# rfonod/geo-trax

Hardware: AMD Instinct MI355X
Metric: 4K frames/sec through detect+stabilize+track (higher is better)
Workload: dtype f32 (split-f16x3 MFMA)

## Files before the change

### geo-trax_amd/csrc/detector.cpp

```cpp
#include "detector.hpp"
#include "split_format.hpp"

#include <algorithm>
#include <cmath>

namespace gtx {

Detector::Detector(gtx_ctx* ctx, const gtx_det_config& cfg)
    : DetectorBase(ctx, cfg, cfg.half ? DT_F16 : (cfg.fp32_split ? DT_F32S : DT_F32), dtype_size(cfg.half ? DT_F16 : DT_F32),
                   cfg.half ? DT_F16 : DT_F32),
      trunk_(*this, ops_, cfg.half ? DT_F16 : DT_F32) {
  dtype_ = cfg.half ? DT_F16 : DT_F32;
  es_ = dtype_size(dtype_);
  lb_ = letterbox_geometry(cfg.frame_h, cfg.frame_w, cfg.imgsz, cfg.rect != 0, 32);
  GTX_CHECK(lb_.net_h % 32 == 0 && lb_.net_w % 32 == 0, "network input %dx%d is not stride aligned", lb_.net_h, lb_.net_w);
}

Detector::~Detector() {
  if (h_feats_) (void)hipHostFree(h_feats_);
  if (h_count_) (void)hipHostFree(h_count_);
}

std::unique_ptr<NetRuntime> Detector::make_exact() const {
  gtx_det_config c = cfg_;
// ... 16 lines not shown
  const YoloTrunk::Levels trunk = trunk_.build(img_);
  const std::vector<View>& lvl_in = trunk.in;
  const std::vector<float>& strides = trunk.strides;
  det_pfx_ = trunk.det_pfx;
  const int nl = (int)lvl_in.size();
  GTX_CHECK(nl <= kMaxLevels, "internal: %d Detect levels", nl);
  const bool has_o2o = has(det_pfx_ + ".one2one_cv2.0.0.conv.weight");
  end2end_ = cfg_.end2end != 0;
  GTX_CHECK(!end2end_ || has_o2o, "end2end: the checkpoint has no one-to-one head (%s.one2one_cv2 / one2one_cv3): only a YOLOv10 file has", det_pfx_.c_str());
  GTX_CHECK(!end2end_ || !cfg_.obj_feats, "end2end: obj_feats (ReID `model: auto`) is not implemented for the one-to-one head");
  const std::string box_br = end2end_ ? ".one2one_cv2." : ".cv2.", cls_br = end2end_ ? ".one2one_cv3." : ".cv3.";
  GTX_CHECK(has(det_pfx_ + box_br + "0.0.conv.weight") && has(det_pfx_ + cls_br + "0.2.weight"),
            "%s: the checkpoint holds no %s / %s tensors (a fused YOLOv10 export keeps the one-to-one head only: run it with end2end)", det_pfx_.c_str(),
            box_br.substr(1, box_br.size() - 2).c_str(), cls_br.substr(1, cls_br.size() - 2).c_str());

  std::vector<Op> st1, st2;
  const bool dw_cls = trunk.dw_cls;
  std::vector<Op> dw_a, pw_a, dw_b;
  head_ = HeadParams{};
  head_.n_levels = nl;
  head_.nc = cfg_.nc;
  head_.conf = cfg_.conf;
  head_.class_mask[0] = head_.class_mask[1] = cfg_.n_classes == 0 ? ~0ull : 0ull;
  for (int i = 0; i < cfg_.n_classes; ++i)
    if (cfg_.classes[i] >= 0 && cfg_.classes[i] < 128) head_.class_mask[cfg_.classes[i] >> 6] |= 1ull << (cfg_.classes[i] & 63);
  int anchor = 0;
  for (int l = 0; l < nl; ++l) {
    const std::string b2 = det_pfx_ + box_br + std::to_string(l), b3 = det_pfx_ + cls_br + std::to_string(l);
    const HostTensor &w20 = tensor(b2 + ".0.conv.weight"), &w30 = tensor(b3 + (dw_cls ? ".1.1.conv.weight" : ".0.conv.weight"));
    const int cb = (int)w20.shape[0], cc = (int)w30.shape[0], cin = (int)w20.shape[1];
    GTX_CHECK(cin == lvl_in[l].c && (dw_cls || (int)w30.shape[1] == cin), "Detect level %d input channels", l);
    Op o1, o2, o3;
// ... 100 lines not shown
      return a.dtype == b.dtype && a.ks == b.ks && a.stride == b.stride && a.bn == b.bn && a.kc == b.kc &&
             a.variant == b.variant && a.th == b.th && a.tw == b.tw;
    };
    auto add = [&](std::vector<Op>& stage, const char* name, const Op& o) {
      for (Op& g : stage)
        if (same(g.cfg, o.cfg) && g.grp.count < kMaxGroup) { g.grp.p[g.grp.count++] = o.grp.p[0]; return; }
      Op g;
      g.kind = Op::CONV;
      g.name = stage.empty() ? std::string(name) : std::string(name) + "." + std::to_string(stage.size());
      g.cfg = o.cfg;
      g.grp.p[g.grp.count++] = o.grp.p[0];
      stage.push_back(g);
    };
    std::vector<Op> d1, d2;
    for (int l = 0; l < nl; ++l) {
      Op o1 = head_ops_[l][0];
      const Op &o2 = head_ops_[l][1], &o3 = head_ops_[l][2];
      if (sparse_on_) {
        const ConvProblem full = o1.grp.p[0];
        const int cb = head_.lv[l].cb, cc = head_.lv[l].cc;
        const size_t tile_bytes = (size_t)(full.Cin / o1.cfg.kc) * 9 * 64 * 128;
        SparseBoxLevel& S = sparse_.lv[l];
        S.in = full.in; S.H = full.H; S.W = full.W; S.cstride = full.in_cstride; S.coff = full.in_coff; S.cin = full.Cin;
        S.w1 = full.wpack; S.b1 = full.bias; S.sc1 = full.acc_scale;
        S.w2 = o2.grp.p[0].wpack; S.b2 = o2.grp.p[0].bias; S.sc2 = o2.grp.p[0].acc_scale;
        S.anchor_begin = head_.lv[l].anchor_begin;
        S.wb = head_.lv[l].wb; S.bb = head_.lv[l].bb; S.stride = head_.lv[l].stride;
        GTX_CHECK(full.bias && o2.grp.p[0].bias && o2.grp.p[0].Cin == 64 && o2.grp.p[0].Cout == 64, "sparse box branch: unexpected Detect box layers");
        Op box1 = o1;
        box1.grp.p[0].Cout = cb;
        add(d1, (det_pfx_ + ".box1").c_str(), box1);
        add(d2, (det_pfx_ + ".box2").c_str(), o2);
        if (dw_cls) {
          add(st1, (det_pfx_ + ".stage1").c_str(), pw_a[l]);
          add(st2, (det_pfx_ + ".stage2").c_str(), o3);
          continue;
        }
        ConvProblem& p = o1.grp.p[0];
        p.wpack = static_cast<const char*>(full.wpack) + tile_bytes;
        p.bias = full.bias + 64;
        p.Cout = cc;
        p.out_coff = full.out_coff + cb;
        add(st1, (det_pfx_ + ".stage1").c_str(), o1);
        add(st2, (det_pfx_ + ".stage2").c_str(), o3);
      } else {
        if (dw_cls) add(st1, (det_pfx_ + ".stage1").c_str(), pw_a[l]);
        add(st1, (det_pfx_ + ".stage1").c_str(), o1);
        add(st2, (det_pfx_ + ".stage2").c_str(), o2);
        add(st2, (det_pfx_ + ".stage2").c_str(), o3);
      }
    }
    if (sparse_on_) {
      sparse_.n_levels = nl;
      for (std::vector<Op>* stage : {&d1, &d2})
        for (Op& g : *stage) { g.family = conv_kernel_name(g.cfg); dense_box_ops_.push_back(g); }
    }
  }
  feat_levels_ = FeatLevels{};
  if (cfg_.obj_feats) {
    feat_levels_.n_levels = nl;
    feat_levels_.dim = lvl_in[0].c;
    for (int l = 1; l < nl; ++l) feat_levels_.dim = std::min(feat_levels_.dim, lvl_in[l].c);
    for (int l = 0; l < nl; ++l) {
      feat_levels_.feat[l] = lvl_in[l].ptr; feat_levels_.h[l] = lvl_in[l].h; feat_levels_.w[l] = lvl_in[l].w;
      feat_levels_.cstride[l] = lvl_in[l].cstride; feat_levels_.coff[l] = lvl_in[l].coff; feat_levels_.c[l] = lvl_in[l].c;
      feat_levels_.anchor_begin[l] = head_.lv[l].anchor_begin;
      GTX_CHECK(lvl_in[l].c % feat_levels_.dim == 0, "obj_feats: Detect input %d has %d channels, not a multiple of %d", l, lvl_in[l].c, feat_levels_.dim);
    }
  }
  for (std::vector<Op>* stage : {&st1, &st2}) {
    for (const Op& d : stage == &st1 ? dw_a : dw_b) ops_.push_back(d);
    for (Op& g : *stage) {
      g.family = conv_kernel_name(g.cfg);
      ops_.push_back(g);
    }
  }
}

void Detector::set_batch(int nb) {
  if (nb == cur_nb_) return;
  set_batch_ops(ops_, nb, es_, pad_skip_on_);
  cur_nb_ = nb;
}

void Detector::plan_pad_skip() {
  pad_skip_rows_ = pad_skip_total_ = 0;
  struct Rows { int lo, hi; };
  std::map<const void*, Rows> dep;
  std::set<const void*> full;
  struct Writer { int c0, c1; Op* op; int member; };
  std::map<const void*, std::vector<Writer>> writers;
// ... 301 lines not shown
```

### geo-trax_amd/csrc/detector.hpp

```cpp
#pragma once
#include <map>
#include <memory>
#include <set>
#include <string>
#include <vector>

#include "yolo_trunk.hpp"

namespace gtx {

class Detector : public DetectorBase {
 public:
  Detector(gtx_ctx* ctx, const gtx_det_config& cfg);
  ~Detector() override;
  void finalize() override;
  void raw_output(int b, float* out, int* n_anchors, bool logits = false) override;
  void layer_output(int b, const std::string& layer, float* out, int* h, int* w, int* c) override;
  void features(int b, float* out, int cap, int* n, int* dim) const override;
  void pad_skip(int* on, int* skipped, int* total) const override {
    if (on) *on = (!exact_ && pad_skip_on_) ? 1 : 0;
    if (skipped) *skipped = pad_skip_rows_;
    if (total) *total = pad_skip_total_;
  }
  void sparse_box(int* on, int* overflows) const override {
    if (on) *on = (!exact_ && sparse_on_) ? 1 : 0;
    if (overflows) *overflows = sparse_overflows_;
  }

 private:
  size_t op_count() const override { return ops_.size(); }
  const OpInfo& op_info(size_t i) const override { return ops_[i]; }
  void launch_op(size_t i, int nb, hipStream_t s) override { run_op(ops_[i], nb, s); }
  std::unique_ptr<NetRuntime> make_exact() const override;
  void release_graph() override { ops_.clear(); trunk_.clear(); }
  View head_conv(const std::string& name, const View& x, const View* out_slice);
  void build_graph();
  void run_op(const Op& op, int nb, hipStream_t s);
  void run_post(int nb, hipStream_t s) override;
  void after_pass(int nb) override;
  void set_batch(int nb) override;

  int dtype_;
  size_t es_;
  std::vector<Op> ops_;
  YoloTrunk trunk_;
  int force_kc_ = 0;
  int force_bn_ = 0;
// ... 1 lines not shown
  HeadParams head_{};
  NmsBuffers nms_{};
  bool end2end_ = false;
  NmsBuffers sel_{};
  float* v10_scores_ = nullptr;
  static constexpr int kSelCap = 304;
  DevBuf raw_;
  bool plain_out_ = false;
  FeatLevels feat_levels_{};
  static constexpr int kSparseCap = 8192;
  bool sparse_on_ = false;
  SparseBox sparse_{};
  Op head_ops_[kMaxLevels][3];
  std::string det_pfx_ = "model.22";
  std::vector<Op> dense_box_ops_;
  bool dense_head_valid_ = false;
  int* h_count_ = nullptr;
  int sparse_overflows_ = 0;
  void run_dense_box(hipStream_t s);
  bool pad_skip_on_ = false;
  int pad_skip_rows_ = 0, pad_skip_total_ = 0;
  void plan_pad_skip();
  void prime_pad_skip();
  float* d_feats_ = nullptr;
  float* h_feats_ = nullptr;
  std::vector<float> c_feats_;
  std::vector<int> c_feat_n_;
};

}
// ... 1 lines not shown
```

### geo-trax_amd/csrc/gtx_api.cpp

```cpp
#include <chrono>
#include <cmath>
#include <cstring>
#include <memory>
#include <string>

#include "../../include/gtx.h"
#include "api_guard.hpp"
#include "common.hpp"
#include "detector.hpp"
#include "draw.hpp"
#include "rtdetr.hpp"
#include "geometry.hpp"
#include "ecc.hpp"
#include "gmc.hpp"
#include "gmc_feat.hpp"
#include "jpeg.hpp"
#include "jpeg_enc.hpp"
#include "jpeg_entropy.hpp"
#include "register.hpp"
#include "sift.hpp"
#include "sift_stab.hpp"
#include "stabilizer.hpp"
#include "tracker.hpp"

// ... 384 lines not shown
                            float* conf, int* cls, float speed_ms[3]) {
  return guarded([&] {
    need(det, "det"); need(frame_dptr, "frame"); need(n_out, "n_out"); need(xyxy, "xyxy"); need(conf, "conf"); need(cls, "cls");
    det->impl->live()->detect_dev(frame_dptr, 1, h, w, n_out, xyxy, conf, cls, speed_ms);
  });
}
int gtx_detector_detect_batch_dev(gtx_detector* det, const void* frames_dptr, int nb, int h, int w, int* n_out,
                                  float* xyxy, float* conf, int* cls, float speed_ms[3]) {
  return guarded([&] {
    need(det, "det"); need(frames_dptr, "frames"); need(n_out, "n_out"); need(xyxy, "xyxy"); need(conf, "conf"); need(cls, "cls");
    det->impl->live()->detect_dev(frames_dptr, nb, h, w, n_out, xyxy, conf, cls, speed_ms);
  });
}
int gtx_detector_submit_dev(gtx_detector* det, const void* frames_dptr, int nb, int h, int w) {
  return guarded([&] { need(det, "det"); need(frames_dptr, "frames"); det->impl->live()->submit_dev(frames_dptr, nb, h, w); });
}
int gtx_detector_collect(gtx_detector* det, int* n_out, float* xyxy, float* conf, int* cls, float speed_ms[3]) {
  return guarded([&] {
    need(det, "det"); need(n_out, "n_out"); need(xyxy, "xyxy"); need(conf, "conf"); need(cls, "cls");
    det->impl->live()->collect(n_out, xyxy, conf, cls, speed_ms);
  });
}
const void* gtx_detector_gray(gtx_detector* det, int b, int* gray_h, int* gray_w) {
  if (!det) return nullptr;
  return det->impl->live()->gray(b, gray_h, gray_w);
}
int gtx_detector_raw_output(gtx_detector* det, int b, float* out, int* n_anchors) {
  return guarded([&] { need(det, "det"); need(out, "out"); det->impl->live()->raw_output(b, out, n_anchors); });
}
int gtx_detector_raw_logits(gtx_detector* det, int b, float* out, int* n_anchors) {
// ... 580 lines not shown
```

### geo-trax_amd/csrc/net_runtime.cpp

```cpp
#include "net_runtime.hpp"
#include "split_format.hpp"

#include <array>
#include <deque>
#include <functional>
#include <mutex>

namespace gtx {

void KernelTable::add(const std::string& label, int n, float t, double f, double b) {
  auto it = idx.find(label);
  size_t k;
  if (it == idx.end()) {
    k = names.size();
    idx[label] = k;
    names.push_back(label);
    launches.push_back(0); ms.push_back(0.f); flops.push_back(0.0); bytes.push_back(0.0);
  } else {
    k = it->second;
  }
  launches[k] += n;
  ms[k] += t;
  flops[k] += f;
  bytes[k] += b;
}

NetRuntime::~NetRuntime() {
  if (h_sat_) (void)hipHostFree(h_sat_);
}

void NetRuntime::set_tensor(const std::string& name, const float* data, int ndim, const int64_t* shape) {
  GTX_CHECK(!finalized_, "set_tensor after finalize");
  HostTensor t;
  size_t n = 1;
  for (int i = 0; i < ndim; ++i) {
    t.shape.push_back(shape[i]);
    n *= (size_t)shape[i];
  }
  t.data.assign(data, data + n);
  tensors_[name] = std::move(t);
}

// ... 38 lines not shown
}

View NetRuntime::new_view(int h, int w, int c, bool plain) {
  View v;
  v.n = max_batch_;
  v.h = h;
  v.w = w;
  v.cstride = c;
  v.coff = 0;
  v.c = c;
  v.plain = plain;
  v.ptr = alloc((size_t)v.n * h * w * c * view_es_);
  return v;
}

void NetRuntime::run_ops(int nb, hipStream_t s, hipEvent_t* ev) {
  const size_t n = op_count();
  for (size_t i = 0; i < n; ++i) {
    if (ev) GTX_HIP(hipEventRecord(ev[i], s));
    launch_op(i, nb, s);
  }
  if (ev) GTX_HIP(hipEventRecord(ev[n], s));
}

namespace {
struct PackedWeights {
  std::vector<uint8_t> bytes;
  float acc_scale = 1.f;
  std::vector<float> source;
};
std::shared_ptr<const PackedWeights> packed_weights(const float* w, size_t n, int cout, int cin, const ConvConfig& cfg,
                                                    const std::function<PackedWeights()>& make) {
  static std::mutex mu;
  static std::map<std::array<uint64_t, 4>, std::shared_ptr<const PackedWeights>> cache;
  uint64_t h = 1469598103934665603ull;
  const uint64_t* q = reinterpret_cast<const uint64_t*>(w);
  for (size_t i = 0; i < n / 2; ++i) h = (h ^ q[i]) * 1099511628211ull;
// ... 196 lines not shown
  GTX_HIP(hipSetDevice(ctx_->device));
  GTX_HIP(hipEventSynchronize(ev_[3]));
  in_flight_ = false;
  collected_gray_slot_ = gray_slot_;
  if (h_sat_ && *h_sat_) {
    sat_seen_ = true;
    if (can_fall_back()) {
      flight_traced_ = false;
      fall_back_to_exact();
      if (trace_every_ > 0) live()->set_trace(trace_every_);
      return live()->detect_dev(cur_frames_, flight_nb_, cfg_.frame_h, cfg_.frame_w, n_out, xyxy, conf, cls, speed_ms);
    }
  }
  if (flight_traced_) {
    for (size_t i = 0; i < op_count(); ++i) {
      float t = 0.f;
      GTX_HIP(hipEventElapsedTime(&t, trace_ev_[i], trace_ev_[i + 1]));
      trace_ms_[i] += t;
      trace_n_[i] += 1;
      trace_flops_[i] += op_info(i).flops;
      trace_bytes_[i] += op_info(i).bytes;
    }
    flight_traced_ = false;
  }
  after_pass(flight_nb_);
  for (int b = 0; b < flight_nb_; ++b) {
    const int n = h_out_n_[b];
    n_out[b] = n;
    const float* rows = h_out_rows_ + (size_t)b * cfg_.max_det * 6;
    for (int i = 0; i < n; ++i) {
      float* bx = xyxy + ((size_t)b * cfg_.max_det + i) * 4;
      bx[0] = rows[i * 6 + 0]; bx[1] = rows[i * 6 + 1]; bx[2] = rows[i * 6 + 2]; bx[3] = rows[i * 6 + 3];
      conf[(size_t)b * cfg_.max_det + i] = rows[i * 6 + 4];
      cls[(size_t)b * cfg_.max_det + i] = (int)rows[i * 6 + 5];
    }
  }
  if (speed_ms)
    for (int i = 0; i < 3; ++i) GTX_HIP(hipEventElapsedTime(&speed_ms[i], ev_[i], ev_[i + 1]));
}

void DetectorBase::detect_dev(const void* frames, int nb, int h, int w, int* n_out, float* xyxy, float* conf, int* cls, float speed_ms[3]) {
  submit_dev(frames, nb, h, w);
  collect(n_out, xyxy, conf, cls, speed_ms);
}

void DetectorBase::detect_host(const uint8_t* frame, int h, int w, int* n_out, float* xyxy, float* conf, int* cls, float speed_ms[3]) {
  GTX_CHECK(finalized_, "detector not finalized");
  GTX_HIP(hipSetDevice(ctx_->device));
  const size_t bytes = (size_t)h * w * 3;
  if (frame_stage_.bytes < bytes) frame_stage_.alloc(bytes);
  GTX_HIP(hipEventRecord(ev_up_[0], ctx_->stream));
  GTX_HIP(hipMemcpyAsync(frame_stage_.p, frame, bytes, hipMemcpyHostToDevice, ctx_->stream));
  GTX_HIP(hipEventRecord(ev_up_[1], ctx_->stream));
// ... 20 lines not shown
  KernelTable table{names, launches, ms, flops, bytes, {}};
  time_ops(nb, iters, [&](size_t i, float t) {
    const OpInfo& op = op_info(i);
    const std::string n = std::to_string(i);
    table.add(per_op ? std::string(n.size() < 3 ? 3 - n.size() : 0, '0') + n + " " + op.name : op.family, 1, t, op.flops, op.bytes);
  });
}

void DetectorBase::set_trace(int every_n) {
  GTX_CHECK(finalized_ && every_n >= 0, "set_trace: detector not finalized or bad period");
  GTX_CHECK(!in_flight_, "set_trace while a batch is in flight");
  trace_every_ = every_n;
  trace_count_ = 0;
  const size_t n = op_count();
  if (every_n > 0 && trace_ev_.empty()) {
    trace_ev_.resize(n + 1);
    for (auto& e : trace_ev_) GTX_HIP(hipEventCreate(&e));
  }
  trace_ms_.assign(n, 0.0);
  trace_n_.assign(n, 0);
  trace_flops_.assign(n, 0.0);
  trace_bytes_.assign(n, 0.0);
}

void DetectorBase::trace_report(std::vector<std::string>& names, std::vector<int>& launches, std::vector<float>& ms,
                                std::vector<double>& flops, std::vector<double>& bytes) {
  KernelTable table{names, launches, ms, flops, bytes, {}};
  const size_t n = op_count();
  for (size_t i = 0; i < n && i < trace_n_.size(); ++i)
    if (trace_n_[i] > 0) table.add(op_info(i).family, trace_n_[i], (float)trace_ms_[i], trace_flops_[i], trace_bytes_[i]);
  trace_ms_.assign(n, 0.0);
// ... 7 lines not shown
```

### geo-trax_amd/csrc/net_runtime.hpp

```cpp
#pragma once
#include <map>
#include <memory>
#include <string>
#include <vector>

#include "../../include/gtx.h"
#include "common.hpp"
#include "conv_igemm.hpp"
#include "det_kernels.hpp"

struct gtx_ctx {
  int device = 0;
  hipStream_t stream = nullptr;
  hipDeviceProp_t prop{};
  void* orb_op_state = nullptr;
  ~gtx_ctx() {
    if (orb_op_state) (void)hipFree(orb_op_state);
    if (stream) (void)hipStreamDestroy(stream);
  }
};

namespace gtx {

struct HostTensor {
// ... 31 lines not shown
  void add(const std::string& label, int n, float t, double f, double b);
};

class YoloTrunk;

class NetRuntime {
 public:
  NetRuntime(gtx_ctx* ctx, int fmt, size_t view_es, int max_batch) : ctx_(ctx), fmt_(fmt), view_es_(view_es), max_batch_(max_batch) {}
  virtual ~NetRuntime();
  NetRuntime(const NetRuntime&) = delete;
  NetRuntime& operator=(const NetRuntime&) = delete;
  friend class YoloTrunk;
  void set_tensor(const std::string& name, const float* data, int ndim, const int64_t* shape);
  bool saturated(bool clear);
  bool fell_back() const { return exact_ != nullptr; }
  virtual void finalize() = 0;

 protected:
  virtual size_t op_count() const = 0;
  virtual const OpInfo& op_info(size_t i) const = 0;
  virtual void launch_op(size_t i, int nb, hipStream_t s) = 0;
  virtual void set_batch(int nb) = 0;
  void run_ops(int nb, hipStream_t s, hipEvent_t* ev);
  template <class F> void time_ops(int nb, int iters, F fold);

  const HostTensor& tensor(const std::string& name) const;
  bool has(const std::string& name) const { return tensors_.count(name) != 0; }
  const float* bias_of(const std::string& name, int cout) const;
  void* alloc(size_t bytes);
  float* upload(const std::vector<float>& v);
  View new_view(int h, int w, int c, bool plain = false);

  struct ConvArgs {
    int stride = 1, act = 1;
    const View* out_slice = nullptr;
    const View* residual = nullptr;
    bool plain_out = false;
    int force_kc = 0, force_bn = 0;
// ... 39 lines not shown
  gtx_ctx* ctx_;
  int fmt_;
  size_t view_es_;
  int max_batch_;
  bool finalized_ = false;
  int cur_nb_ = 0;
  std::map<std::string, HostTensor> tensors_;
  std::vector<DevBuf> bufs_;
  std::map<std::string, View> layer_views_;
  std::unique_ptr<NetRuntime> exact_;
  int* sat_dev_ = nullptr;
  int* h_sat_ = nullptr;
  bool sat_seen_ = false;

 private:
  View conv_problem(const std::string& name, const float* w_oihw, int cout, int cin, int ks, const float* bias, const View& x,
                    const ConvArgs& a, ConvConfig& cfg, ConvProblem& p);
};

template <class F>
void NetRuntime::time_ops(int nb, int iters, F fold) {
  hipStream_t s = ctx_->stream;
  set_batch(nb);
  const size_t n = op_count();
  std::vector<hipEvent_t> ev(n + 1);
  for (auto& e : ev) GTX_HIP(hipEventCreate(&e));
  for (int it = 0; it < iters; ++it) {
    run_ops(nb, s, ev.data());
    GTX_HIP(hipStreamSynchronize(s));
    for (size_t i = 0; i < n; ++i) {
      float t = 0.f;
      GTX_HIP(hipEventElapsedTime(&t, ev[i], ev[i + 1]));
      fold(i, t);
    }
  }
  for (auto& e : ev) (void)hipEventDestroy(e);
}

class DetectorBase : public NetRuntime {
 public:
  DetectorBase(gtx_ctx* ctx, const gtx_det_config& cfg, int fmt, size_t view_es, int in_dtype);
  ~DetectorBase() override;
  DetectorBase* live() { return live_as<DetectorBase>(); }
  void input_size(int* h, int* w) const { *h = lb_.net_h; *w = lb_.net_w; }
  void detect_dev(const void* frames, int nb, int h, int w, int* n_out, float* xyxy, float* conf, int* cls, float speed_ms[3]);
  void submit_dev(const void* frames, int nb, int h, int w);
  void collect(int* n_out, float* xyxy, float* conf, int* cls, float speed_ms[3]);
  void detect_host(const uint8_t* frame, int h, int w, int* n_out, float* xyxy, float* conf, int* cls, float speed_ms[3]);
  const void* gray(int b, int* gh, int* gw) const;
  virtual void raw_output(int b, float* out, int* n_anchors, bool logits = false) = 0;
  virtual void layer_output(int b, const std::string& layer, float* out, int* h, int* w, int* c) = 0;
  void profile(int nb, int iters, std::vector<std::string>& names, std::vector<int>& launches, std::vector<float>& ms,
               std::vector<double>& flops, std::vector<double>& bytes);
  void set_trace(int every_n);
  void trace_report(std::vector<std::string>& names, std::vector<int>& launches, std::vector<float>& ms, std::vector<double>& flops,
                    std::vector<double>& bytes);
  virtual void features(int b, float* out, int cap, int* n, int* dim) const = 0;
  virtual void pad_skip(int* on, int* skipped, int* total) const = 0;
  virtual void sparse_box(int* on, int* overflows) const = 0;

  static constexpr int kGrayRing = 16;

// ... 37 lines not shown
```

### geo-trax_amd/csrc/yolo_trunk.hpp

```cpp
#pragma once
#include <string>
#include <vector>

#include "net_runtime.hpp"
#include "yolo_tables.hpp"

namespace gtx {

struct Op : OpInfo {
  enum Kind { CONV, STEM, POOL, UPSAMPLE, DWCONV, ATTN, POOLDOWN } kind = CONV;
  ConvGroup grp{};
  ConvConfig cfg{};
  View in, out;
  const float* w27 = nullptr;
  const float* bias = nullptr;
  const void* wpk = nullptr;
  float stem_scale = 1.f;
  const void* front_wpk = nullptr;
  float front_scale = 1.f;
  const float* dw_w = nullptr;
  const float* dw_bias = nullptr;
  int dw_act = 0, heads = 0;
  int dw_k = 3, dw_stride = 1;
  View dw_res;
  View out2;
  int* sat = nullptr;
  int ty_first[kMaxGroup] = {0}, ty_count[kMaxGroup] = {0};
};

void set_batch_ops(std::vector<Op>& ops, int nb, size_t es, bool pad_skip_on);

class YoloTrunk {
 public:
  YoloTrunk(NetRuntime& net, std::vector<Op>& ops, int dtype) : net_(net), ops_(ops), dtype_(dtype) {}

  struct Levels {
    std::vector<View> in;
    std::vector<float> strides;
    std::string det_pfx;
    bool dw_cls = false;
  };
  TrunkGraph choose_graph() const;
// ... 41 lines not shown
```

### geo-trax_amd/geotrax_amd/_lib.py

```python
from __future__ import annotations

import ctypes as C
import os
from pathlib import Path

import numpy as np

_HERE = Path(__file__).resolve().parent
LIB_PATH = Path(os.environ.get("GTX_LIB", _HERE / "libgtx.so"))


class GtxError(RuntimeError):
    def __init__(self, code: int, msg: str):
        super().__init__(f"libgtx error {code}: {msg}")
        self.code = code


class ConvDesc(C.Structure):
    _fields_ = [(n, C.c_int) for n in (
        "dtype", "n", "h", "w", "cin", "cout", "ksize", "stride", "act",
        "in_cstride", "in_coff", "out_cstride", "out_coff", "has_residual")]


class ConvFused(C.Structure):
# ... 183 lines not shown
    "gtx_sift_stab_keypoints": (C.c_int, [_P, C.c_int, C.c_int, C.POINTER(C.c_int), _P, _P, _P]),
    "gtx_sift_stab_pairs": (C.c_int, [_P, C.c_int, C.POINTER(C.c_int), _P]),
    "gtx_sift_stab_counters": (C.c_int, [_P, _P]),
    "gtx_op_match_2nn": (C.c_int, [_P, _P, C.c_int, _P, C.c_int, _P, _P, _P, _P, C.c_int, _P]),
    "gtx_op_preprocess": (C.c_int, [_P, C.c_int, _P, C.c_int, C.c_int, C.c_int, C.c_int, _P, _P, C.c_int, C.c_int]),
    "gtx_detector_create": (C.c_int, [_P, C.POINTER(DetConfig), C.POINTER(_P)]),
    "gtx_detector_destroy": (None, [_P]),
    "gtx_detector_set_tensor": (C.c_int, [_P, C.c_char_p, _P, C.c_int, C.POINTER(C.c_int64)]),
    "gtx_detector_finalize": (C.c_int, [_P]),
    "gtx_detector_input_size": (C.c_int, [_P, C.POINTER(C.c_int), C.POINTER(C.c_int)]),
    "gtx_detector_detect": (C.c_int, [_P, _P, C.c_int, C.c_int, _P, _P, _P, _P, _P]),
    "gtx_detector_detect_dev": (C.c_int, [_P, _P, C.c_int, C.c_int, _P, _P, _P, _P, _P]),
    "gtx_detector_detect_batch_dev": (C.c_int, [_P, _P, C.c_int, C.c_int, C.c_int, _P, _P, _P, _P, _P]),
    "gtx_detector_submit_dev": (C.c_int, [_P, _P, C.c_int, C.c_int, C.c_int]),
    "gtx_detector_collect": (C.c_int, [_P, _P, _P, _P, _P, _P]),
    "gtx_detector_gray": (_P, [_P, C.c_int, C.POINTER(C.c_int), C.POINTER(C.c_int)]),
    "gtx_detector_raw_output": (C.c_int, [_P, C.c_int, _P, C.POINTER(C.c_int)]),
    "gtx_detector_raw_logits": (C.c_int, [_P, C.c_int, _P, C.POINTER(C.c_int)]),
    "gtx_detector_layer_output": (C.c_int, [_P, C.c_int, C.c_char_p, _P, C.POINTER(C.c_int), C.POINTER(C.c_int), C.POINTER(C.c_int)]),
    "gtx_detector_saturated": (C.c_int, [_P, C.c_int, C.POINTER(C.c_int)]),
    "gtx_detector_fell_back": (C.c_int, [_P, C.POINTER(C.c_int)]),
    "gtx_detector_pad_skip": (C.c_int, [_P, C.POINTER(C.c_int), C.POINTER(C.c_int), C.POINTER(C.c_int)]),
    "gtx_detector_sparse_box": (C.c_int, [_P, C.POINTER(C.c_int), C.POINTER(C.c_int)]),
    "gtx_detector_features": (C.c_int, [_P, C.c_int, _P, C.c_int, C.POINTER(C.c_int), C.POINTER(C.c_int)]),
    "gtx_detector_trace": (C.c_int, [_P, C.c_int]),
    "gtx_detector_profile": (C.c_int, [_P, C.c_int, C.c_int, C.c_int, _P, _P, _P, _P, _P, C.POINTER(C.c_int)]),
    "gtx_embedder_create": (C.c_int, [_P, C.c_int, C.c_int, C.c_int, C.POINTER(_P)]),
    "gtx_embedder_destroy": (None, [_P]),
    "gtx_embedder_set_tensor": (C.c_int, [_P, C.c_char_p, _P, C.c_int, C.POINTER(C.c_int64)]),
    "gtx_embedder_finalize": (C.c_int, [_P]),
# ... 183 lines not shown
```

### geo-trax_amd/geotrax_amd/detector.py

```python
from __future__ import annotations

import ctypes as C
import logging
import os
from dataclasses import dataclass

import numpy as np

from . import _lib
from ._lib import DetConfig, check, ptr

logger = logging.getLogger(__name__)


FP32_SPLIT_DEFAULT = True


@dataclass
class Detections:
    xyxy: np.ndarray
    conf: np.ndarray
    cls: np.ndarray
    speed: dict
    feats: np.ndarray | None = None
# ... 106 lines not shown
            return False
        f = C.c_int()
        check(self.ctx.lib.gtx_detector_saturated(self.handle, int(clear), C.byref(f)))
        return bool(f.value)

    def pad_skip(self) -> tuple[bool, int, int]:
        on, sk, tot = C.c_int(), C.c_int(), C.c_int()
        check(self.ctx.lib.gtx_detector_pad_skip(self.handle, C.byref(on), C.byref(sk), C.byref(tot)))
        return bool(on.value), int(sk.value), int(tot.value)

    def sparse_box(self) -> tuple[bool, int]:
        on, over = C.c_int(), C.c_int()
        check(self.ctx.lib.gtx_detector_sparse_box(self.handle, C.byref(on), C.byref(over)))
        return bool(on.value), int(over.value)

    def fell_back(self) -> bool:
        f = C.c_int()
        check(self.ctx.lib.gtx_detector_fell_back(self.handle, C.byref(f)))
        return bool(f.value)

    def _collect(self, nb: int) -> list[Detections]:
        if self.fp32_split and not self._sat_warned and self.saturated():
            self._sat_warned = True
            if self.fell_back():
                logger.warning("activations beyond fp16's range (|x| > 65504) reached the split-f16x3 convolutions: the batch was re-run with the "
                               "exact-fp32 MFMA convolutions and the detector stays on them for the rest of the run (same results as fp32_split: "
                               "false, at its speed); set fp32_split: false for this checkpoint to skip the detour")
            else:
                logger.warning("activations beyond fp16's range (|x| > 65504) were clamped by the split-f16x3 convolutions and GTX_SAT_FALLBACK=0 "
                               "keeps them: detections differ from an fp32 run of this checkpoint")
# ... 24 lines not shown
    def detect_dev(self, frames_dptr: int, nb: int = 1) -> list[Detections]:
        h, w = self.frame_hw
        check(self.ctx.lib.gtx_detector_detect_batch_dev(self.handle, C.c_void_p(frames_dptr), nb, h, w, ptr(self._n),
                                                         ptr(self._xyxy), ptr(self._conf), ptr(self._cls), ptr(self._speed)))
        return self._collect(nb)

    def submit_dev(self, frames_dptr: int, nb: int = 1) -> None:
        h, w = self.frame_hw
        check(self.ctx.lib.gtx_detector_submit_dev(self.handle, C.c_void_p(frames_dptr), nb, h, w))
        self._flight = nb

    def collect(self) -> list[Detections]:
        check(self.ctx.lib.gtx_detector_collect(self.handle, ptr(self._n), ptr(self._xyxy), ptr(self._conf), ptr(self._cls),
                                                ptr(self._speed)))
        return self._collect(self._flight)

    def gray_dptr(self, b: int = 0) -> tuple[int, int, int]:
        gh, gw = C.c_int(), C.c_int()
        p = self.ctx.lib.gtx_detector_gray(self.handle, b, C.byref(gh), C.byref(gw))
        return p, gh.value, gw.value

    def raw_output(self, b: int = 0, logits: bool = False) -> np.ndarray:
        na = C.c_int()
        h, w = self.net_hw
        anchors = (h // 8) * (w // 8) + (h // 16) * (w // 16) + (h // 32) * (w // 32)
        if self.p2:
            anchors += (h // 4) * (w // 4)
        if self.rtdetr:
            anchors = self.n_queries
        out = np.zeros((anchors, 4 + self.nc), np.float32)
# ... 41 lines not shown
```

### geo-trax_amd/geotrax_amd/engine.py

```python
from __future__ import annotations

import collections
import ctypes as C
import os
import queue
import threading
import time
import weakref
from dataclasses import dataclass

import numpy as np

from . import _lib
from .detector import Detector
from .geometry import warp_boxes
from .sift_stabilizer import SiftStabilizer, resident
from .stabilizer import Stabilizer
from .tracker import Tracker


@dataclass
class FrameResult:
    index: int
    xyxy: np.ndarray
# ... 60 lines not shown
                dets_left -= 1
            elif null_left:
                order.append("n")
                null_left = False
            else:
                order.append("x")
        elif busy:
            order.append(busy.pop(0))
        else:
            order.append("x")
    if null_left:
        order.append("n")
    while any(q < n_dets for q in queue_of_streams(order + ["?", "?"], n_queues)[-2:]):
        order.append("x")
    return order


class PacedSource:
    paced = True

    def __init__(self, batches):
        self._it = batches

    def __iter__(self):
        return iter(self._it)


class StreamPlan:
    _plans: dict = {}
    _lock = threading.Lock()
# ... 54 lines not shown
                cand = _lib.Context(self.device, self.p_det)
                o1, o2 = self.overlap(dets[0][1], cand)
                if o2 < 1.5 * o1 and all(self.overlap(other[1], cand)[1] < 1.5 * o1 for other in dets[1:] if other is not ent):
                    log.warning(f"stream plan: two detector streams of device {self.device} ran one after the other ({two:.2f} ms for two "
                                f"{one:.2f} ms kernels): this HIP runtime does not place streams the way the plan assumes; "
                                "a replacement stream that does overlap was found and is used instead")
                    spares.append(ent[1])
                    ent[1] = cand
                    break
                spares.append(cand)
            else:
                log.warning(f"stream plan: two detector streams of device {self.device} share a hardware queue ({two:.2f} ms for two {one:.2f} ms "
                            "kernels) and no replacement stream overlaps: expect 15-20 % lower frame rates (GPU_MAX_HW_QUEUES, GTX_ENGINE_ORDER)")
            self.ctxs.extend(["x", c, True] for c in spares)

    def take(self, role: str, holder=None) -> _lib.Context:
        with self._lock:
            for ent in self.ctxs:
                if ent[0] == role and (ent[2] is None or (ent[2] is not True and ent[2]() is None)):
                    ent[2] = weakref.ref(holder) if holder is not None else True
                    return ent[1]
            ctx = _lib.Context(self.device, self.p_det if role == "d" else self.p_stab if role in ("s", "g") else 0)
            self.ctxs.append([role, ctx, weakref.ref(holder) if holder is not None else True])
            return ctx

    def give_back(self, ctx: _lib.Context) -> None:
        with self._lock:
            for ent in self.ctxs:
                if ent[1] is ctx:
                    ent[2] = None
# ... 20 lines not shown
            det_kw = dict(det_kw, obj_feats=True)
            if any(not getattr(d, "obj_feats", False) for d in self.dets):
                raise ValueError("the tracker associates on appearance vectors (with_reid): adopted detectors must be built with obj_feats=True")
        self.gmc = None
        self.stabs = []
        self.plan = StreamPlan.get(self.device, n_dets, n_stab)
        self._taken = []

        def take(role):
            ctx = self.plan.take(role, holder=self)
            self._taken.append(ctx)
            return ctx

        while len(self.dets) < n_dets:
            self.dets.append(Detector(weights, self.frame_hw, max_batch=self.B, ctx=take("d"), **det_kw))
        stab_cls = stab_cls or stabilizer_class(stab_kw)
        while len(self.stabs) < n_stab:
            self.stabs.append(stab_cls(self.frame_hw, ctx=take("s"), **stab_kw))
        if self.reid_tensors is not None:
            from .reid import ReIDEncoder

            for d in self.dets:
                self.encoders[id(d)] = ReIDEncoder(self.reid_tensors, ctx=d.ctx, max_crops=min(d.max_det * self.B, 256),
                                                     fp32_split=det_kw.get("fp32_split"))
        self.feeder_ctx = take("f") if feeder_stream else None
        if gmc:
            from .gmc import make_gmc

            self.gmc = make_gmc(self.frame_hw, method=gmc if isinstance(gmc, str) else "sparseOptFlow", ctx=take("g"),
                                **(gmc_kw or {}))
# ... 373 lines not shown
```

### include/gtx.h

```cpp
#ifndef GTX_H_
#define GTX_H_

#include <stddef.h>
#include <stdint.h>

#ifdef __cplusplus
extern "C" {
#endif

#define GTX_ABI_VERSION 14

typedef enum gtx_status {
  GTX_OK = 0,
  GTX_ERR_INVALID = -1,
  GTX_ERR_HIP = -2,
  GTX_ERR_UNSUPPORTED = -3,
  GTX_ERR_STATE = -4,
  GTX_ERR_INTERNAL = -5
} gtx_status;

typedef enum gtx_dtype { GTX_F16 = 0, GTX_F32 = 1, GTX_F32S = 2 } gtx_dtype;

typedef struct gtx_ctx gtx_ctx;
typedef struct gtx_detector gtx_detector;
// ... 208 lines not shown
int gtx_detector_set_tensor(gtx_detector* det, const char* name, const float* data, int ndim,
                            const int64_t* shape);
int gtx_detector_finalize(gtx_detector* det);
int gtx_detector_input_size(gtx_detector* det, int* net_h, int* net_w);

int gtx_detector_detect(gtx_detector* det, const uint8_t* frame_bgr, int h, int w, int* n_out,
                        float* xyxy, float* conf, int* cls, float speed_ms[3]);
int gtx_detector_detect_dev(gtx_detector* det, const void* frame_dptr, int h, int w, int* n_out,
                            float* xyxy, float* conf, int* cls, float speed_ms[3]);
int gtx_detector_detect_batch_dev(gtx_detector* det, const void* frames_dptr, int nb, int h, int w,
                                  int* n_out, float* xyxy, float* conf, int* cls,
                                  float speed_ms[3]);
int gtx_detector_submit_dev(gtx_detector* det, const void* frames_dptr, int nb, int h, int w);
int gtx_detector_collect(gtx_detector* det, int* n_out, float* xyxy, float* conf, int* cls,
                         float speed_ms[3]);
const void* gtx_detector_gray(gtx_detector* det, int b, int* gray_h, int* gray_w);
int gtx_detector_raw_output(gtx_detector* det, int b, float* out, int* n_anchors);
int gtx_detector_raw_logits(gtx_detector* det, int b, float* out, int* n_anchors);
int gtx_detector_layer_output(gtx_detector* det, int b, const char* layer, float* out,
                              int* h, int* w, int* c);
int gtx_detector_saturated(gtx_detector* det, int clear, int* flag);
int gtx_detector_fell_back(gtx_detector* det, int* fell_back);
int gtx_detector_sparse_box(gtx_detector* det, int* on, int* overflows);
int gtx_detector_pad_skip(gtx_detector* det, int* on, int* skipped, int* total);
int gtx_detector_features(gtx_detector* det, int b, float* out, int cap, int* n, int* dim);

int gtx_detector_trace(gtx_detector* det, int every_n);
int gtx_detector_profile(gtx_detector* det, int nb, int iters, int cap, char* names,
                         int* launches, float* total_ms, double* flops, double* bytes,
                         int* n_families);
// ... 288 lines not shown
```

Measured before the change: 1145.

## Overlap per-level Detect head convs with the trunk on a side stream

Finds the last trunk op that writes each Detect input level and inserts that level's head convs right after it. When the level is ready before the trunk finishes, the head convs run on a second non-blocking stream, forked and joined with events. This lets the P3/P4 head work run alongside the remaining trunk layers instead of waiting for the whole trunk. It adds a buffer-clash check, per-op event timing across streams, hardware-queue padding in the engine so the side streams don't collide with other detectors, and a chain_dev API for multi-pass submission. The costs are extra fork/join synchronisation and possible contention for compute units.

```diff
diff --git a/geo-trax_amd/csrc/detector.cpp b/geo-trax_amd/csrc/detector.cpp
--- a/geo-trax_amd/csrc/detector.cpp
+++ b/geo-trax_amd/csrc/detector.cpp
@@ -54,8 +54,29 @@
             "%s: the checkpoint holds no %s / %s tensors (a fused YOLOv10 export keeps the one-to-one head only: run it with end2end)", det_pfx_.c_str(),
             box_br.substr(1, box_br.size() - 2).c_str(), cls_br.substr(1, cls_br.size() - 2).c_str());
 
-  std::vector<Op> st1, st2;
   const bool dw_cls = trunk.dw_cls;
+  const size_t n_trunk = ops_.size();
+  std::vector<size_t> ready(nl, n_trunk - 1);
+  head_overlap_ = env_flag("GTX_HEAD_OVERLAP", true) && !dw_cls && !end2end_ && nl > 1;
+  for (int l = 0; l < nl && head_overlap_; ++l) {
+    const View& v = lvl_in[l];
+    auto hit = [&](const void* p, int c0, int c) { return p == v.ptr && c0 < v.coff + v.c && v.coff < c0 + c; };
+    int last = -1;
+    for (size_t i = 0; i < n_trunk; ++i) {
+      const Op& o = ops_[i];
+      bool w = false;
+      if (o.kind == Op::CONV) {
+        for (int k = 0; k < o.grp.count; ++k) w = w || hit(o.grp.p[k].out, o.grp.p[k].out_coff, o.grp.p[k].Cout);
+      } else {
+        w = hit(o.out.ptr, o.out.coff, o.out.c) || (o.out2.ptr && hit(o.out2.ptr, o.out2.coff, o.out2.c));
+      }
+      if (w) last = (int)i;
+    }
+    if (last < 0) head_overlap_ = false;
+    else ready[l] = (size_t)last;
+  }
+  struct Branch { size_t after; std::string sfx; std::vector<Op> st1, st2; };
+  std::vector<Branch> branches;
   std::vector<Op> dw_a, pw_a, dw_b;
   head_ = HeadParams{};
   head_.n_levels = nl;
@@ -186,6 +207,16 @@
     };
     std::vector<Op> d1, d2;
     for (int l = 0; l < nl; ++l) {
+      const size_t after = head_overlap_ ? ready[l] : n_trunk - 1;
+      size_t bi = 0;
+      while (bi < branches.size() && branches[bi].after != after) ++bi;
+      if (bi == branches.size()) {
+        int p = 0;
+        while ((1 << (p + 1)) <= (int)strides[l]) ++p;
+        branches.push_back(Branch{after, head_overlap_ ? ".P" + std::to_string(p) : std::string(), {}, {}});
+      }
+      std::vector<Op>&st1 = branches[bi].st1, &st2 = branches[bi].st2;
+      const std::string n1 = det_pfx_ + ".stage1" + branches[bi].sfx, n2 = det_pfx_ + ".stage2" + branches[bi].sfx;
       Op o1 = head_ops_[l][0];
       const Op &o2 = head_ops_[l][1], &o3 = head_ops_[l][2];
       if (sparse_on_) {
@@ -204,8 +235,8 @@
         add(d1, (det_pfx_ + ".box1").c_str(), box1);
         add(d2, (det_pfx_ + ".box2").c_str(), o2);
         if (dw_cls) {
-          add(st1, (det_pfx_ + ".stage1").c_str(), pw_a[l]);
-          add(st2, (det_pfx_ + ".stage2").c_str(), o3);
+          add(st1, n1.c_str(), pw_a[l]);
+          add(st2, n2.c_str(), o3);
           continue;
         }
         ConvProblem& p = o1.grp.p[0];
@@ -213,13 +244,13 @@
         p.bias = full.bias + 64;
         p.Cout = cc;
         p.out_coff = full.out_coff + cb;
-        add(st1, (det_pfx_ + ".stage1").c_str(), o1);
-        add(st2, (det_pfx_ + ".stage2").c_str(), o3);
+        add(st1, n1.c_str(), o1);
+        add(st2, n2.c_str(), o3);
       } else {
-        if (dw_cls) add(st1, (det_pfx_ + ".stage1").c_str(), pw_a[l]);
-        add(st1, (det_pfx_ + ".stage1").c_str(), o1);
-        add(st2, (det_pfx_ + ".stage2").c_str(), o2);
-        add(st2, (det_pfx_ + ".stage2").c_str(), o3);
+        if (dw_cls) add(st1, n1.c_str(), pw_a[l]);
+        add(st1, n1.c_str(), o1);
+        add(st2, n2.c_str(), o2);
+        add(st2, n2.c_str(), o3);
       }
     }
     if (sparse_on_) {
@@ -240,13 +271,39 @@
       GTX_CHECK(lvl_in[l].c % feat_levels_.dim == 0, "obj_feats: Detect input %d has %d channels, not a multiple of %d", l, lvl_in[l].c, feat_levels_.dim);
     }
   }
-  for (std::vector<Op>* stage : {&st1, &st2}) {
-    for (const Op& d : stage == &st1 ? dw_a : dw_b) ops_.push_back(d);
-    for (Op& g : *stage) {
-      g.family = conv_kernel_name(g.cfg);
-      ops_.push_back(g);
-    }
-  }
+  std::sort(branches.begin(), branches.end(), [](const Branch& a, const Branch& b) { return a.after > b.after; });
+  for (Branch& br : branches) {
+    std::vector<Op> seq;
+    for (std::vector<Op>* stage : {&br.st1, &br.st2}) {
+      for (const Op& d : stage == &br.st1 ? dw_a : dw_b) seq.push_back(d);
+      for (Op& g : *stage) {
+        g.family = conv_kernel_name(g.cfg);
+        g.side = br.after + 1 < n_trunk;
+        seq.push_back(g);
+      }
+    }
+    ops_.insert(ops_.begin() + (long)br.after + 1, seq.begin(), seq.end());
+  }
+  bool any_side = false;
+  for (size_t i = 0; i < ops_.size(); ++i) {
+    if (!ops_[i].side) continue;
+    any_side = true;
+    for (int k = 0; k < ops_[i].grp.count; ++k) {
+      const ConvProblem& q = ops_[i].grp.p[k];
+      for (size_t j = 0; j < ops_.size(); ++j) {
+        const Op& o = ops_[j];
+        if (o.side) continue;
+        bool clash = o.kind != Op::CONV && (o.in.ptr == q.out || o.out.ptr == q.out || o.out2.ptr == q.out || (j > i && (o.out.ptr == q.in || o.out2.ptr == q.in)));
+        for (int m = 0; m < o.grp.count && o.kind == Op::CONV; ++m) {
+          const ConvProblem& t = o.grp.p[m];
+          clash = clash || t.in == q.out || t.out == q.out || t.res == q.out || t.in2 == q.out;
+          clash = clash || (j > i && t.out == q.in && t.out_coff < q.in_coff + q.Cin && q.in_coff < t.out_coff + t.Cout);
+        }
+        GTX_CHECK(!clash, "internal: %s on the side stream shares a buffer with %s", ops_[i].name.c_str(), o.name.c_str());
+      }
+    }
+  }
+  if (any_side) (void)side_stream();
 }
 
 void Detector::set_batch(int nb) {
diff --git a/geo-trax_amd/csrc/detector.hpp b/geo-trax_amd/csrc/detector.hpp
--- a/geo-trax_amd/csrc/detector.hpp
+++ b/geo-trax_amd/csrc/detector.hpp
@@ -31,6 +31,7 @@
   size_t op_count() const override { return ops_.size(); }
   const OpInfo& op_info(size_t i) const override { return ops_[i]; }
   void launch_op(size_t i, int nb, hipStream_t s) override { run_op(ops_[i], nb, s); }
+  bool op_on_side(size_t i) const override { return ops_[i].side; }
   std::unique_ptr<NetRuntime> make_exact() const override;
   void release_graph() override { ops_.clear(); trunk_.clear(); }
   View head_conv(const std::string& name, const View& x, const View* out_slice);
@@ -62,6 +63,7 @@
   Op head_ops_[kMaxLevels][3];
   std::string det_pfx_ = "model.22";
   std::vector<Op> dense_box_ops_;
+  bool head_overlap_ = false;
   bool dense_head_valid_ = false;
   int* h_count_ = nullptr;
   int sparse_overflows_ = 0;
diff --git a/geo-trax_amd/csrc/gtx_api.cpp b/geo-trax_amd/csrc/gtx_api.cpp
--- a/geo-trax_amd/csrc/gtx_api.cpp
+++ b/geo-trax_amd/csrc/gtx_api.cpp
@@ -422,6 +422,15 @@
 }
 int gtx_detector_submit_dev(gtx_detector* det, const void* frames_dptr, int nb, int h, int w) {
   return guarded([&] { need(det, "det"); need(frames_dptr, "frames"); det->impl->live()->submit_dev(frames_dptr, nb, h, w); });
+}
+int gtx_detector_head_overlap(gtx_detector* det, int* on) {
+  return guarded([&] { need(det, "det"); need(on, "on"); *on = det->impl->has_side_stream() ? 1 : 0; });
+}
+int gtx_detector_chain_dev(gtx_detector* det, const void* const* frames_dptr, int n_passes, int nb, int h, int w, int* n_out, float* rows) {
+  return guarded([&] {
+    need(det, "det"); need(frames_dptr, "frames"); need(n_out, "n_out"); need(rows, "rows");
+    det->impl->live()->chain_dev(frames_dptr, n_passes, nb, h, w, n_out, rows);
+  });
 }
 int gtx_detector_collect(gtx_detector* det, int* n_out, float* xyxy, float* conf, int* cls, float speed_ms[3]) {
   return guarded([&] {
diff --git a/geo-trax_amd/csrc/net_runtime.cpp b/geo-trax_amd/csrc/net_runtime.cpp
--- a/geo-trax_amd/csrc/net_runtime.cpp
+++ b/geo-trax_amd/csrc/net_runtime.cpp
@@ -26,6 +26,12 @@
 }
 
 NetRuntime::~NetRuntime() {
+  if (side_) {
+    (void)hipStreamSynchronize(side_);
+    (void)hipStreamDestroy(side_);
+  }
+  for (auto& e : fork_ev_) (void)hipEventDestroy(e);
+  if (join_ev_) (void)hipEventDestroy(join_ev_);
   if (h_sat_) (void)hipHostFree(h_sat_);
 }
 
@@ -94,13 +100,66 @@
   return v;
 }
 
+hipStream_t NetRuntime::side_stream() {
+  if (!side_) {
+    GTX_HIP(hipSetDevice(ctx_->device));
+    GTX_HIP(hipStreamCreateWithFlags(&side_, hipStreamNonBlocking));
+    GTX_HIP(hipEventCreateWithFlags(&join_ev_, hipEventDisableTiming));
+  }
+  return side_;
+}
+
+size_t NetRuntime::event_count() const {
+  const size_t n = op_count();
+  size_t k = 0;
+  for (size_t i = 0; i < n; ++i) k += op_on_side(i) ? 1 : 0;
+  return n + 1 + k;
+}
+
+float NetRuntime::op_elapsed(const hipEvent_t* ev, size_t i) const {
+  const size_t n = op_count();
+  size_t end = n;
+  if (op_on_side(i)) {
+    end = n + 1;
+    for (size_t j = 0; j < i; ++j) end += op_on_side(j) ? 1 : 0;
+  } else {
+    for (size_t j = i + 1; j < n; ++j)
+      if (!op_on_side(j)) { end = j; break; }
+  }
+  float t = 0.f;
+  GTX_HIP(hipEventElapsedTime(&t, ev[i], ev[end]));
+  return t;
+}
+
 void NetRuntime::run_ops(int nb, hipStream_t s, hipEvent_t* ev) {
   const size_t n = op_count();
+  size_t branch = 0, side_ops = 0;
   for (size_t i = 0; i < n; ++i) {
-    if (ev) GTX_HIP(hipEventRecord(ev[i], s));
-    launch_op(i, nb, s);
+    if (!op_on_side(i)) {
+      if (ev) GTX_HIP(hipEventRecord(ev[i], s));
+      launch_op(i, nb, s);
+      continue;
+    }
+    hipStream_t side = side_stream();
+    if (i == 0 || !op_on_side(i - 1)) {
+      if (branch == fork_ev_.size()) {
+        fork_ev_.push_back(nullptr);
+        GTX_HIP(hipEventCreateWithFlags(&fork_ev_.back(), hipEventDisableTiming));
+      }
+      GTX_HIP(hipEventRecord(fork_ev_[branch], s));
+      GTX_HIP(hipStreamWaitEvent(side, fork_ev_[branch], 0));
+      ++branch;
+    }
+    if (ev) GTX_HIP(hipEventRecord(ev[i], side));
+    launch_op(i, nb, side);
+    if (ev) GTX_HIP(hipEventRecord(ev[n + 1 + side_ops], side));
+    ++side_ops;
   }
   if (ev) GTX_HIP(hipEventRecord(ev[n], s));
+  if (side_ops) {
+    GTX_HIP(hipEventRecord(join_ev_, side_));
+    GTX_HIP(hipStreamWaitEvent(s, join_ev_, 0));
+  }
 }
 
 namespace {
@@ -327,9 +386,7 @@
   }
   if (flight_traced_) {
     for (size_t i = 0; i < op_count(); ++i) {
-      float t = 0.f;
-      GTX_HIP(hipEventElapsedTime(&t, trace_ev_[i], trace_ev_[i + 1]));
-      trace_ms_[i] += t;
+      trace_ms_[i] += op_elapsed(trace_ev_.data(), i);
       trace_n_[i] += 1;
       trace_flops_[i] += op_info(i).flops;
       trace_bytes_[i] += op_info(i).bytes;
@@ -350,6 +407,52 @@
   }
   if (speed_ms)
     for (int i = 0; i < 3; ++i) GTX_HIP(hipEventElapsedTime(&speed_ms[i], ev_[i], ev_[i + 1]));
+}
+
+void DetectorBase::chain_dev(const void* const* frames, int n_passes, int nb, int h, int w, int* n_out, float* rows) {
+  GTX_CHECK(n_passes >= 1 && n_passes <= kGrayRing, "chain of %d passes outside [1,%d]", n_passes, kGrayRing);
+  GTX_CHECK(!in_flight_, "chain while a batch is in flight: call collect first");
+  for (int k = 0; k < n_passes; ++k) GTX_CHECK(frames[k], "frames[%d] is NULL", k);
+  GTX_HIP(hipSetDevice(ctx_->device));
+  const size_t per_n = (size_t)cfg_.max_batch, per_rows = (size_t)6 * cfg_.max_batch * cfg_.max_det;
+  int* const keep_n = h_out_n_;
+  float* const keep_rows = h_out_rows_;
+  int* pn = nullptr;
+  float* pr = nullptr;
+  GTX_HIP(hipHostMalloc((void**)&pn, sizeof(int) * per_n * n_passes));
+  if (hipHostMalloc((void**)&pr, sizeof(float) * per_rows * n_passes) != hipSuccess) {
+    (void)hipHostFree(pn);
+    fail(-1, "chain: no pinned memory for %d passes", n_passes);
+  }
+  auto restore = [&] {
+    h_out_n_ = keep_n;
+    h_out_rows_ = keep_rows;
+    in_flight_ = false;
+    (void)hipStreamSynchronize(ctx_->stream);
+  };
+  try {
+    for (int k = 0; k < n_passes; ++k) {
+      h_out_n_ = pn + per_n * k;
+      h_out_rows_ = pr + per_rows * k;
+      submit_dev(frames[k], nb, h, w);
+      in_flight_ = false;
+      flight_traced_ = false;
+    }
+  } catch (...) {
+    restore();
+    (void)hipHostFree(pn);
+    (void)hipHostFree(pr);
+    throw;
+  }
+  restore();
+  for (int k = 0; k < n_passes; ++k)
+    for (int b = 0; b < nb; ++b) {
+      const int n = pn[per_n * k + b];
+      n_out[(size_t)k * nb + b] = n;
+      memcpy(rows + ((size_t)k * nb + b) * cfg_.max_det * 6, pr + per_rows * k + (size_t)b * cfg_.max_det * 6, sizeof(float) * 6 * std::max(n, 0));
+    }
+  (void)hipHostFree(pn);
+  (void)hipHostFree(pr);
 }
 
 void DetectorBase::detect_dev(const void* frames, int nb, int h, int w, int* n_out, float* xyxy, float* conf, int* cls, float speed_ms[3]) {
@@ -400,7 +503,7 @@
   trace_count_ = 0;
   const size_t n = op_count();
   if (every_n > 0 && trace_ev_.empty()) {
-    trace_ev_.resize(n + 1);
+    trace_ev_.resize(event_count());
     for (auto& e : trace_ev_) GTX_HIP(hipEventCreate(&e));
   }
   trace_ms_.assign(n, 0.0);
diff --git a/geo-trax_amd/csrc/net_runtime.hpp b/geo-trax_amd/csrc/net_runtime.hpp
--- a/geo-trax_amd/csrc/net_runtime.hpp
+++ b/geo-trax_amd/csrc/net_runtime.hpp
@@ -69,6 +69,7 @@
   void set_tensor(const std::string& name, const float* data, int ndim, const int64_t* shape);
   bool saturated(bool clear);
   bool fell_back() const { return exact_ != nullptr; }
+  bool has_side_stream() const { return side_ != nullptr; }
   virtual void finalize() = 0;
 
  protected:
@@ -76,7 +77,11 @@
   virtual const OpInfo& op_info(size_t i) const = 0;
   virtual void launch_op(size_t i, int nb, hipStream_t s) = 0;
   virtual void set_batch(int nb) = 0;
+  virtual bool op_on_side(size_t i) const { (void)i; return false; }
   void run_ops(int nb, hipStream_t s, hipEvent_t* ev);
+  size_t event_count() const;
+  float op_elapsed(const hipEvent_t* ev, size_t i) const;
+  hipStream_t side_stream();
   template <class F> void time_ops(int nb, int iters, F fold);
 
   const HostTensor& tensor(const std::string& name) const;
@@ -146,6 +151,9 @@
   bool sat_seen_ = false;
 
  private:
+  hipStream_t side_ = nullptr;
+  std::vector<hipEvent_t> fork_ev_;
+  hipEvent_t join_ev_ = nullptr;
   View conv_problem(const std::string& name, const float* w_oihw, int cout, int cin, int ks, const float* bias, const View& x,
                     const ConvArgs& a, ConvConfig& cfg, ConvProblem& p);
 };
@@ -155,16 +163,12 @@
   hipStream_t s = ctx_->stream;
   set_batch(nb);
   const size_t n = op_count();
-  std::vector<hipEvent_t> ev(n + 1);
+  std::vector<hipEvent_t> ev(event_count());
   for (auto& e : ev) GTX_HIP(hipEventCreate(&e));
   for (int it = 0; it < iters; ++it) {
     run_ops(nb, s, ev.data());
     GTX_HIP(hipStreamSynchronize(s));
-    for (size_t i = 0; i < n; ++i) {
-      float t = 0.f;
-      GTX_HIP(hipEventElapsedTime(&t, ev[i], ev[i + 1]));
-      fold(i, t);
-    }
+    for (size_t i = 0; i < n; ++i) fold(i, op_elapsed(ev.data(), i));
   }
   for (auto& e : ev) (void)hipEventDestroy(e);
 }
@@ -178,6 +182,7 @@
   void detect_dev(const void* frames, int nb, int h, int w, int* n_out, float* xyxy, float* conf, int* cls, float speed_ms[3]);
   void submit_dev(const void* frames, int nb, int h, int w);
   void collect(int* n_out, float* xyxy, float* conf, int* cls, float speed_ms[3]);
+  void chain_dev(const void* const* frames, int n_passes, int nb, int h, int w, int* n_out, float* rows);
   void detect_host(const uint8_t* frame, int h, int w, int* n_out, float* xyxy, float* conf, int* cls, float speed_ms[3]);
   const void* gray(int b, int* gh, int* gw) const;
   virtual void raw_output(int b, float* out, int* n_anchors, bool logits = false) = 0;
diff --git a/geo-trax_amd/csrc/yolo_trunk.hpp b/geo-trax_amd/csrc/yolo_trunk.hpp
--- a/geo-trax_amd/csrc/yolo_trunk.hpp
+++ b/geo-trax_amd/csrc/yolo_trunk.hpp
@@ -26,6 +26,7 @@
   View out2;
   int* sat = nullptr;
   int ty_first[kMaxGroup] = {0}, ty_count[kMaxGroup] = {0};
+  bool side = false;
 };
 
 void set_batch_ops(std::vector<Op>& ops, int nb, size_t es, bool pad_skip_on);
diff --git a/geo-trax_amd/geotrax_amd/_lib.py b/geo-trax_amd/geotrax_amd/_lib.py
--- a/geo-trax_amd/geotrax_amd/_lib.py
+++ b/geo-trax_amd/geotrax_amd/_lib.py
@@ -221,6 +221,8 @@
     "gtx_detector_detect_batch_dev": (C.c_int, [_P, _P, C.c_int, C.c_int, C.c_int, _P, _P, _P, _P, _P]),
     "gtx_detector_submit_dev": (C.c_int, [_P, _P, C.c_int, C.c_int, C.c_int]),
     "gtx_detector_collect": (C.c_int, [_P, _P, _P, _P, _P, _P]),
+    "gtx_detector_head_overlap": (C.c_int, [_P, C.POINTER(C.c_int)]),
+    "gtx_detector_chain_dev": (C.c_int, [_P, _P, C.c_int, C.c_int, C.c_int, C.c_int, _P, _P]),
     "gtx_detector_gray": (_P, [_P, C.c_int, C.POINTER(C.c_int), C.POINTER(C.c_int)]),
     "gtx_detector_raw_output": (C.c_int, [_P, C.c_int, _P, C.POINTER(C.c_int)]),
     "gtx_detector_raw_logits": (C.c_int, [_P, C.c_int, _P, C.POINTER(C.c_int)]),
diff --git a/geo-trax_amd/geotrax_amd/detector.py b/geo-trax_amd/geotrax_amd/detector.py
--- a/geo-trax_amd/geotrax_amd/detector.py
+++ b/geo-trax_amd/geotrax_amd/detector.py
@@ -144,6 +144,11 @@
         check(self.ctx.lib.gtx_detector_sparse_box(self.handle, C.byref(on), C.byref(over)))
         return bool(on.value), int(over.value)
 
+    def head_overlap(self) -> bool:
+        on = C.c_int()
+        check(self.ctx.lib.gtx_detector_head_overlap(self.handle, C.byref(on)))
+        return bool(on.value)
+
     def fell_back(self) -> bool:
         f = C.c_int()
         check(self.ctx.lib.gtx_detector_fell_back(self.handle, C.byref(f)))
@@ -198,6 +203,15 @@
         check(self.ctx.lib.gtx_detector_collect(self.handle, ptr(self._n), ptr(self._xyxy), ptr(self._conf), ptr(self._cls),
                                                 ptr(self._speed)))
         return self._collect(self._flight)
+
+    def chain_dev(self, frames_dptrs: list[int], nb: int = 1) -> list[list[np.ndarray]]:
+        h, w = self.frame_hw
+        k = len(frames_dptrs)
+        arr = (C.c_void_p * k)(*frames_dptrs)
+        n = np.zeros((k, nb), np.int32)
+        rows = np.zeros((k, nb, self.max_det, 6), np.float32)
+        check(self.ctx.lib.gtx_detector_chain_dev(self.handle, arr, k, nb, h, w, ptr(n), ptr(rows)))
+        return [[rows[i, b, :n[i, b]].copy() for b in range(nb)] for i in range(k)]
 
     def gray_dptr(self, b: int = 0) -> tuple[int, int, int]:
         gh, gw = C.c_int(), C.c_int()
diff --git a/geo-trax_amd/geotrax_amd/engine.py b/geo-trax_amd/geotrax_amd/engine.py
--- a/geo-trax_amd/geotrax_amd/engine.py
+++ b/geo-trax_amd/geotrax_amd/engine.py
@@ -98,6 +98,18 @@
     while any(q < n_dets for q in queue_of_streams(order + ["?", "?"], n_queues)[-2:]):
         order.append("x")
     return order
+
+
+def side_stream_padding(order: list[str], n_side: int, n_queues: int = 4) -> int:
+    seq = list(order) + ["h"] * n_side
+    det_q = {q for t, q in zip(seq, queue_of_streams(seq, n_queues)) if t == "d"}
+    if n_side <= 0 or len(det_q) >= n_queues:
+        return 0
+    n = 0
+    while n < 4 * n_queues and any(q in det_q for q in queue_of_streams(seq + ["?", "?"], n_queues)[-2:]):
+        seq.append("x")
+        n += 1
+    return n
 
 
 class PacedSource:
@@ -182,6 +194,18 @@
                             "kernels) and no replacement stream overlaps: expect 15-20 % lower frame rates (GPU_MAX_HW_QUEUES, GTX_ENGINE_ORDER)")
             self.ctxs.extend(["x", c, True] for c in spares)
 
+    def pad_side_streams(self, n_side: int) -> None:
+        with self._lock:
+            if n_side <= 0 or getattr(self, "_side_padded", False):
+                return
+            self._side_padded = True
+            try:
+                n_queues = max(int(os.environ.get("GPU_MAX_HW_QUEUES", "4")), 1)
+            except ValueError:
+                n_queues = 4
+            for _ in range(side_stream_padding(self.order, n_side, n_queues)):
+                self.ctxs.append(["x", _lib.Context(self.device, 0), True])
+
     def take(self, role: str, holder=None) -> _lib.Context:
         with self._lock:
             for ent in self.ctxs:
@@ -232,6 +256,7 @@
 
         while len(self.dets) < n_dets:
             self.dets.append(Detector(weights, self.frame_hw, max_batch=self.B, ctx=take("d"), **det_kw))
+        self.plan.pad_side_streams(sum(1 for d in self.dets if getattr(d, "head_overlap", None) and d.head_overlap()))
         stab_cls = stab_cls or stabilizer_class(stab_kw)
         while len(self.stabs) < n_stab:
             self.stabs.append(stab_cls(self.frame_hw, ctx=take("s"), **stab_kw))
diff --git a/include/gtx.h b/include/gtx.h
--- a/include/gtx.h
+++ b/include/gtx.h
@@ -246,6 +246,9 @@
 int gtx_detector_submit_dev(gtx_detector* det, const void* frames_dptr, int nb, int h, int w);
 int gtx_detector_collect(gtx_detector* det, int* n_out, float* xyxy, float* conf, int* cls,
                          float speed_ms[3]);
+int gtx_detector_chain_dev(gtx_detector* det, const void* const* frames_dptr, int n_passes, int nb, int h, int w,
+                           int* n_out, float* rows);
+int gtx_detector_head_overlap(gtx_detector* det, int* on);
 const void* gtx_detector_gray(gtx_detector* det, int b, int* gray_h, int* gray_w);
 int gtx_detector_raw_output(gtx_detector* det, int b, float* out, int* n_anchors);
 int gtx_detector_raw_logits(gtx_detector* det, int b, float* out, int* n_anchors);
```

After: 1156 (median of 6 runs). No clear change (+0.9%).
